# huttered40/capital

Hardware: AMD Instinct MI355X
Metric: TFLOP/s (whole node) Cholesky n=65536, algorithmic n^3/3, recursive cholinv factor(), inputs resident in HBM (higher is better)
Workload: dtype f64

## Files before the change

### capital_amd/src/alg/cholesky/cholinv/cholinv.h

```cpp
#ifndef CAPITAL_CHOLESKY_CHOLINV_H_
#define CAPITAL_CHOLESKY_CHOLINV_H_

#include "./../../alg.h"
#include "./../../matmult/summa/summa.h"
#include "./policy.h"

#pragma weak capi_dtrmm_thin
#pragma weak capi_dresid_ts

namespace cholesky {

template <class SerializePolicy = policy::cholinv::Serialize, class IntermediatesPolicy = policy::cholinv::SaveIntermediates,
          class BaseCasePolicy = policy::cholinv::NoReplication>
class cholinv : public SerializePolicy, public IntermediatesPolicy, public BaseCasePolicy {
public:
  using SP = SerializePolicy;
  using IP = IntermediatesPolicy;
  using BP = BaseCasePolicy;

  template <typename ScalarT, typename DimensionT>
  class info {
  public:
    using ScalarType = ScalarT;
    using DimensionType = DimensionT;
    using alg_type = cholinv<SerializePolicy, IntermediatesPolicy, BaseCasePolicy>;
    using SP = SerializePolicy;
    using IP = IntermediatesPolicy;
    using BP = BaseCasePolicy;
    info(const info& p) : complete_inv(p.complete_inv), split(p.split), bc_mult_dim(p.bc_mult_dim), dir(p.dir) {}
    info(info&& p) : complete_inv(p.complete_inv), split(p.split), bc_mult_dim(p.bc_mult_dim), dir(p.dir) {}
    info(DimensionType complete_inv, DimensionType split, DimensionType bc_mult_dim, char dir)
        : complete_inv(complete_inv), split(split), bc_mult_dim(bc_mult_dim), dir(dir) {}
    const DimensionType complete_inv, split, bc_mult_dim;
    const char dir;
    matrix<ScalarType, DimensionType, typename SerializePolicy::structure> R, Rinv;
    matrix<ScalarType, DimensionType, rect> Rfull, Rinvfull;
    matmult::arena work;
    DimensionType localDimension = 0, globalDimension = 0, trueLocalDimension = 0, trueGlobalDimension = 0, bcDimension = 0;
    int64_t num_base_cases = 0, num_levels = 0;
    bool solve_with_trsm = false;
    int potrf_info = 0;
    bool zeroed = false;
    const double* input = nullptr;
    DimensionType early_split = 0;
    DimensionType input_lead = 0;
    int la_depth = 0;
    bool factored = false, factored_trsm = false;
    DimensionType top_split = 0;
    matrix<ScalarType, DimensionType, rect> X, SolveW1, SolveW2, SolveRho, SolveD, SolveNorm2;
    std::vector<double> solve_residual_norms;
  };

  template <typename MatrixType, typename ArgType, typename CommType>
  static void factor(const MatrixType& A, ArgType& args, CommType&& CommInfo) {
    CRITTER_START(CI::factor);
    using U = typename ArgType::DimensionType;
    static_assert(std::is_same<typename MatrixType::StructureType, rect>::value, "cholinv::factor takes a rect-structured input block");
    if (!(args.split > 0) || args.dir != 'U') throw std::invalid_argument("cholinv: split > 0 and dir == 'U' required (cholinv.hpp:9)");
    if (CommInfo.d > 1 && CommInfo.d % CommInfo.c) throw std::invalid_argument("cholinv: c must divide d (or d == 1)");
    args.factored = false;
    args.factored_trsm = args.solve_with_trsm;
    args.top_split = 0;
    if (args.solve_with_trsm) { factor_trsm(A, args, CommInfo); args.factored = true; CRITTER_STOP(CI::factor); return; }
    const U localDimension = A.num_rows_local(), globalDimension = A.num_rows_global();
    CAPITAL_CHECK(capi_stream_select(capital::handle(), 0));
    CAPITAL_CHECK(capi_reset_info(capital::handle()));
    args.potrf_info = 0;
    args.R._register_(A.num_columns_global(), A.num_rows_global(), CommInfo.d, CommInfo.d);
    args.Rinv._register_(A.num_columns_global(), A.num_rows_global(), CommInfo.d, CommInfo.d);
    constexpr bool packed = !std::is_same<typename SP::structure, rect>::value;
    if (packed) {
      args.Rfull._register_(A.num_columns_global(), A.num_rows_global(), CommInfo.d, CommInfo.d);
      args.Rinvfull._register_(A.num_columns_global(), A.num_rows_global(), CommInfo.d, CommInfo.d);
    }
    double* R = packed ? args.Rfull.data() : (double*)args.R.data();
    double* Ri = packed ? args.Rinvfull.data() : (double*)args.Rinv.data();
    const U ld = localDimension;
    if (!args.zeroed) {
      capital::dev_zero(R, ld * ld);
      capital::dev_zero(Ri, ld * ld);
      args.zeroed = true;
    }
    U bcDimLocal = (U)(CommInfo.c * CommInfo.d);
    U bcMult = args.bc_mult_dim;
    if (bcMult < 0) { bcMult = -bcMult; for (U i = 0; i < bcMult; ++i) bcDimLocal *= 2; } else { for (U i = 0; i < bcMult; ++i) bcDimLocal /= 2; }
    bcDimLocal = std::max<U>(1, bcDimLocal);
    bcDimLocal = std::min<U>(localDimension, bcDimLocal);
    bcDimLocal = localDimension / bcDimLocal;
    args.localDimension = args.trueLocalDimension = localDimension;
    args.globalDimension = args.trueGlobalDimension = globalDimension;
    args.bcDimension = (U)CommInfo.d * bcDimLocal;
    args.num_base_cases = args.num_levels = 0;

    const U h1 = localDimension >> args.split;
    args.input = A.data();
    args.early_split = 0;
    const bool will_split = !(((localDimension * (U)CommInfo.d) <= args.bcDimension) || (h1 < args.split));
    args.input_lead = 0;
    args.top_split = will_split ? h1 : 0;
    if (will_split && h1 > 0 && h1 < ld) {
      capi_handle_t hh = capital::handle();
      U lead = h1;
      if (args.split == 1 && CommInfo.d == 1 && CommInfo.c == 1) while (lead >= 8192 && lead % 2 == 0 && (lead >> 1) * (U)CommInfo.d > args.bcDimension) lead >>= 1;
      CAPITAL_CHECK(capi_dlacpy(hh, 1, lead, lead, A.data(), ld, R, ld));
      CAPITAL_CHECK(capi_event_record(hh, EV_INPUT_HEAD));
      CAPITAL_CHECK(capi_stream_select(hh, 1));
      CAPITAL_CHECK(capi_event_wait(hh, EV_INPUT_HEAD));
      if (lead < h1) {
        CAPITAL_CHECK(capi_dlacpy(hh, 0, lead, h1 - lead, A.data() + (int64_t)lead * ld, ld, R + (int64_t)lead * ld, ld));
        CAPITAL_CHECK(capi_dlacpy(hh, 1, h1 - lead, h1 - lead, A.data() + lead + (int64_t)lead * ld, ld, R + lead + (int64_t)lead * ld, ld));
        CAPITAL_CHECK(capi_event_record(hh, EV_INPUT_MID));
        args.input_lead = lead;
      }
      CAPITAL_CHECK(capi_dlacpy(hh, 0, h1, ld - h1, A.data() + (int64_t)h1 * ld, ld, R + (int64_t)h1 * ld, ld));
      CAPITAL_CHECK(capi_dlacpy(hh, 1, ld - h1, ld - h1, A.data() + h1 + (int64_t)h1 * ld, ld, R + h1 + (int64_t)h1 * ld, ld));
      CAPITAL_CHECK(capi_event_record(hh, EV_INPUT_REST));
      CAPITAL_CHECK(capi_stream_select(hh, 0));
      args.early_split = h1;
    } else {
      CAPITAL_CHECK(capi_dlacpy(capital::handle(), 1, ld, ld, A.data(), ld, R, ld));
    }


    const bool single = (CommInfo.d == 1 && CommInfo.c == 1);
    capital::launch_rounds_scope rounds(true);
    const U h = localDimension - (localDimension >> args.split);
    const U agg = args.bcDimension;
    int64_t need = single ? (int64_t)h * h + (int64_t)h * h / 3 + 1024 : (int64_t)(CommInfo.d == 1 ? 8 : 12) * h * h + 4 * (int64_t)agg * agg + 4096;
    args.work.reserve(need);

    args.la_depth = 0;
    invoke(args, CommInfo, R, Ri, ld, (U)0, localDimension, globalDimension);

    if (packed) {
      const U e = args.early_split;
      if (e > 0) {
        pack_block(args, CAPI_UPPERTRI, R, (double*)args.R.data(), ld, e, ld, e, ld);
        pack_block(args, CAPI_UPPERTRI, Ri, (double*)args.Rinv.data(), ld, e, ld, e, ld);
        if (args.complete_inv) pack_block(args, CAPI_RECT, Ri, (double*)args.Rinv.data(), ld, e, ld, 0, e);
        CAPITAL_CHECK(capi_event_wait(capital::handle(), EV_EARLY_PACK));
      } else {
        serialize<uppertri, uppertri>::invoke(args.Rfull, args.R, 0, ld, 0, ld, 0, ld, 0, ld);
        serialize<uppertri, uppertri>::invoke(args.Rinvfull, args.Rinv, 0, ld, 0, ld, 0, ld, 0, ld);
      }
    }
    if (!IP::keep_arena) {
      capital::sync();
      args.work.release();
      if (packed) { args.Rfull._destroy_(); args.Rinvfull._destroy_(); args.zeroed = false; }
    }
    CRITTER_STOP(CI::factor);
    CAPITAL_CHECK(capi_get_info(capital::handle(), &args.potrf_info));
    const int failed = capital::ranks_with_nonzero(CommInfo.world, args.potrf_info);
    if (failed != 0)
      throw std::domain_error("cholinv::factor: the matrix is not positive definite (" +
                              (args.potrf_info != 0 ? "non-positive pivot " + std::to_string(args.potrf_info) + " of a diagonal block"
                                                    : std::string("reported by ") + std::to_string(failed) + " other rank(s) of the grid") +
                              "); R and Rinv are not valid");
    args.factored = true;
  }

  template <typename MatrixType, typename ArgType, typename CommType>
  static void solve(const MatrixType& A, const MatrixType& B, ArgType& args, CommType&& CommInfo, int refine = 1, bool residual = true) {
    static_assert(std::is_same<typename MatrixType::StructureType, rect>::value, "cholinv::solve takes rect-structured A and B");
    constexpr bool packed = !std::is_same<typename SP::structure, rect>::value;
    if (CommInfo.size > 1) throw std::logic_error("cholinv::solve is built for one rank: on a grid the factors are element-cyclic (factor there, solve on one rank)");
    if (!&capi_dtrmm_thin || !&capi_dresid_ts) throw std::logic_error("cholinv: this C-ABI library has no capi_dtrmm_thin / capi_dresid_ts: no solve");
    if (!args.factored || args.potrf_info != 0 || !args.R.filled() || (!args.solve_with_trsm && !args.Rinv.filled()))
      throw std::logic_error("cholinv::solve: factor() has not run or did not succeed: there are no valid factors to solve with");
    if (args.factored_trsm != args.solve_with_trsm)
      throw std::logic_error("cholinv::solve: solve_with_trsm was changed after factor(): the resident factors are those of the other mode; factor() again");
    const int64_t n = args.localDimension, r = B.num_columns_global();
    if (r < 1 || B.num_rows_global() != n || B.num_rows_local() != n || A.num_rows_local() != n || A.num_columns_local() != n || refine < 0)
      throw std::invalid_argument("cholinv::solve: B must be n x r with r >= 1 (matrix(r, n, 1, 1)), A the factored matrix, refine >= 0");
    const double* Rfullp = nullptr;
    if (args.solve_with_trsm) {
      Rfullp = packed ? (IP::keep_arena && args.Rfull.filled() ? args.Rfull.data() : nullptr) : (const double*)args.R.data();
      if (!Rfullp)
        throw std::logic_error("cholinv::solve: TRSM mode with Serialize + FlushIntermediates leaves only the packed R, and capi_dtrsm takes full "
                               "storage: use SaveIntermediates or NoSerialize with solve_with_trsm");
    }
    CRITTER_START(CI::solve);
    capi_handle_t h = capital::handle();
    CAPITAL_CHECK(capi_stream_select(h, 0));
    const int64_t W = CAPI_TS_MAX_RHS, h1 = args.top_split;
    const bool blocks = !args.solve_with_trsm && !args.complete_inv && h1 > 0 && h1 < n;
    if (args.X.filled() && args.X.num_columns_local() != r) args.X._destroy_();
    args.X._register_(r, n, 1, 1);
    args.SolveW1._register_(W, n, 1, 1);
    if (blocks) args.SolveW2._register_(W, n, 1, 1);
    if (refine > 0) { args.SolveRho._register_(W, n, 1, 1); args.SolveD._register_(W, n, 1, 1); }
    const double* Rp = (const double*)args.R.data();
    const double* Ip = args.solve_with_trsm ? nullptr : (const double*)args.Rinv.data();
    auto thin = [&](const double* F, int shape, int trans, int64_t i0, int64_t j0, int64_t m, int64_t k, int64_t rb, double alpha, const double* Bp,
                    double beta, double* Cp) {
      const double* Tp = packed ? F + j0 * (j0 + 1) / 2 + i0 : F + i0 + j0 * n;
      CAPITAL_CHECK(capi_dtrmm_thin(h, shape, trans, m, k, rb, alpha, Tp, packed ? 0 : n, packed ? j0 : 0, Bp, n, beta, Cp, n));
    };
    auto apply = [&](const double* Bi, double* Xo, int64_t rb) {
      double* w1 = args.SolveW1.data();
      if (args.solve_with_trsm) {
        CAPITAL_CHECK(capi_dlacpy(h, 0, n, rb, Bi, n, Xo, n));
        CAPITAL_CHECK(capi_dtrsm(h, CAPI_LEFT, CAPI_UPPER, CAPI_TRANS, CAPI_NONUNIT, n, rb, 1.0, Rfullp, n, Xo, n));
        CAPITAL_CHECK(capi_dtrsm(h, CAPI_LEFT, CAPI_UPPER, CAPI_NOTRANS, CAPI_NONUNIT, n, rb, 1.0, Rfullp, n, Xo, n));
      } else if (!blocks) {
        thin(Ip, CAPI_UPPERTRI, CAPI_TRANS, 0, 0, n, n, rb, 1.0, Bi, 0.0, w1);
        thin(Ip, CAPI_UPPERTRI, CAPI_NOTRANS, 0, 0, n, n, rb, 1.0, w1, 0.0, Xo);
      } else {
        const int64_t h2 = n - h1;
        double* w2 = args.SolveW2.data();
        thin(Ip, CAPI_UPPERTRI, CAPI_TRANS, 0, 0, h1, h1, rb, 1.0, Bi, 0.0, w1);
        CAPITAL_CHECK(capi_dlacpy(h, 0, h2, rb, Bi + h1, n, w2 + h1, n));
        thin(Rp, CAPI_RECT, CAPI_TRANS, 0, h1, h1, h2, rb, -1.0, w1, 1.0, w2 + h1);
        thin(Ip, CAPI_UPPERTRI, CAPI_TRANS, h1, h1, h2, h2, rb, 1.0, w2 + h1, 0.0, w1 + h1);
        thin(Ip, CAPI_UPPERTRI, CAPI_NOTRANS, h1, h1, h2, h2, rb, 1.0, w1 + h1, 0.0, Xo + h1);
        thin(Rp, CAPI_RECT, CAPI_NOTRANS, 0, h1, h1, h2, rb, -1.0, Xo + h1, 1.0, w1);
        thin(Ip, CAPI_UPPERTRI, CAPI_NOTRANS, 0, 0, h1, h1, rb, 1.0, w1, 0.0, Xo);
      }
    };
    for (int64_t j = 0; j < r; j += W) {
      const int64_t rb = std::min(W, r - j);
      double* Xj = args.X.data() + j * n;
      const double* Bj = B.data() + j * n;
      apply(Bj, Xj, rb);
      for (int it = 0; it < refine; ++it) {
        CAPITAL_CHECK(capi_dresid_ts(h, n, n, rb, A.data(), n, Xj, n, Bj, n, args.SolveRho.data(), n, nullptr));
        apply(args.SolveRho.data(), args.SolveD.data(), rb);
        CAPITAL_CHECK(capi_dgeadd(h, 0, n, rb, 1.0, args.SolveD.data(), n, 1.0, Xj, n));
      }
    }
    args.solve_residual_norms.clear();
    if (residual) {
      if (args.SolveNorm2.filled() && args.SolveNorm2.num_columns_local() != r) args.SolveNorm2._destroy_();
      args.SolveNorm2._register_(r, 1, 1, 1);
      for (int64_t j = 0; j < r; j += W)
        CAPITAL_CHECK(capi_dresid_ts(h, n, n, std::min(W, r - j), A.data(), n, args.X.data() + j * n, n, B.data() + j * n, n, nullptr, 0,
                                     args.SolveNorm2.data() + j));
      args.solve_residual_norms = args.SolveNorm2.to_host();
      for (double& v : args.solve_residual_norms) v = std::sqrt(v);
    }
    if (!IP::keep_arena) {
      capital::sync();
      args.SolveW1._destroy_(); args.SolveW2._destroy_(); args.SolveRho._destroy_(); args.SolveD._destroy_();
    }
    CRITTER_STOP(CI::solve);
  }

  template <typename MatrixType, typename ArgType, typename CommType>
  static void factor_trsm(const MatrixType& A, ArgType& args, CommType&& CommInfo) {
    using U = typename ArgType::DimensionType;
    capi_handle_t h = capital::handle();
    const U ld = A.num_rows_local();
    CAPITAL_CHECK(capi_stream_select(h, 0));
    CAPITAL_CHECK(capi_reset_info(h));
    args.potrf_info = 0;
    args.R._register_(A.num_columns_global(), A.num_rows_global(), CommInfo.d, CommInfo.d);
    constexpr bool packed = !std::is_same<typename SP::structure, rect>::value;
    if (packed) args.Rfull._register_(A.num_columns_global(), A.num_rows_global(), CommInfo.d, CommInfo.d);
    double* R = packed ? args.Rfull.data() : (double*)args.R.data();
    if (!args.zeroed) { capital::dev_zero(R, ld * ld); args.zeroed = true; }
    CAPITAL_CHECK(capi_dlacpy(h, 1, ld, ld, A.data(), ld, R, ld));
    U bcDimLocal = (U)(CommInfo.c * CommInfo.d), bcMult = args.bc_mult_dim;
    if (bcMult < 0) { bcMult = -bcMult; for (U i = 0; i < bcMult; ++i) bcDimLocal *= 2; } else { for (U i = 0; i < bcMult; ++i) bcDimLocal /= 2; }
    bcDimLocal = ld / std::min<U>(ld, std::max<U>(1, bcDimLocal));
    args.localDimension = args.trueLocalDimension = ld;
    args.globalDimension = args.trueGlobalDimension = A.num_rows_global();
    args.bcDimension = (U)CommInfo.d * bcDimLocal;
    args.num_base_cases = args.num_levels = 0;
    if (CommInfo.d == 1) {
      potrf_rec(args, R, ld, (U)0, ld);
    } else {
      const U hh = ld - (ld >> args.split);
      args.work.reserve((int64_t)32 * hh * hh + 4 * (int64_t)args.bcDimension * args.bcDimension + 4096);
      potrf_rec_grid(args, CommInfo, R, ld, (U)0, ld);
    }
    if (packed) serialize<uppertri, uppertri>::invoke(args.Rfull, args.R, 0, ld, 0, ld, 0, ld, 0, ld);
    CAPITAL_CHECK(capi_get_info(h, &args.potrf_info));
    const int failed = capital::ranks_with_nonzero(CommInfo.world, args.potrf_info);
    if (failed != 0)
      throw std::domain_error("cholinv::factor (TRSM mode): the matrix is not positive definite (non-positive pivot " + std::to_string(args.potrf_info) + " of a diagonal block)");
  }

  template <typename ArgType, typename CommType, typename U>
  static void potrf_rec_grid(ArgType& args, CommType&& t, double* R, U ld, U start, U dim) {
    using matmult::view;
    capi_handle_t h = capital::handle();
    matmult::arena& ws = args.work;
    const int64_t d = (int64_t)t.d, P = (int64_t)t.size, me = (int64_t)t.x + d * (int64_t)t.y;
    const U split1 = dim >> args.split;
    double* R11 = R + start + start * ld;
    if (((dim * (U)t.d) <= args.bcDimension) || (split1 < args.split)) {
      CRITTER_START(CI::factor_diag);
      const int64_t L = dim, agg = L * d;
      const int64_t span = ((start + dim) != args.trueLocalDimension) ? agg : agg - (args.trueLocalDimension * d - args.trueGlobalDimension);
      const int64_t mark = ws.top;
      double* mine = ws.take(L * L);
      double* blocked = ws.take(L * L * d * d);
      double* cyc = ws.take(agg * agg);
      CAPITAL_CHECK(capi_dlacpy(h, 0, L, L, R11, ld, mine, L));
      CAPITAL_CHECK(capi_allgather(t.slice, mine, blocked, L * L));
      util::block_to_cyclic_rect(blocked, cyc, L, L, d);
      CAPITAL_CHECK(capi_dpotrf(h, CAPI_UPPER, span, cyc, agg));
      CAPITAL_CHECK(capi_dtrizero(h, CAPI_UPPER, agg, cyc, agg));
      util::cyclic_to_block_rect(blocked, cyc, L, L, d);
      CAPITAL_CHECK(capi_dlacpy(h, 0, L, L, blocked + me * L * L, L, R11, ld));
      ws.top = mark;
      ++args.num_base_cases;
      CRITTER_STOP(CI::factor_diag);
      return;
    }
    ++args.num_levels;
    const U split2 = dim - split1;
    double* R12 = R + start + (start + split1) * ld;
    view A22{R + (start + split1) + (start + split1) * ld, ld, split2, split2};
    potrf_rec_grid(args, t, R, ld, start, split1);
    CRITTER_START(CI::trsm);
    const int64_t mark = ws.top;
    view W{ws.take((int64_t)split1 * split2), split1, split1, split2};
    {
      const int64_t L1 = split1, L2 = split2, S1 = L1 * d, S2 = L2 * d;
      const int64_t ncw = (((S2 + P - 1) / P) + 1) & ~(int64_t)1, S2p = ncw * P;
      const int64_t inner = ws.top;
      double* Rf = ws.take(S1 * S1);
      double* Xf = ws.take(S1 * S2p);
      double* mine = ws.take(L1 * std::max(L1, L2));
      double* blocked = ws.take(L1 * std::max(L1, L2) * d * d);
      CAPITAL_CHECK(capi_dlacpy(h, 0, L1, L1, R11, ld, mine, L1));
      CAPITAL_CHECK(capi_allgather(t.slice, mine, blocked, L1 * L1));
      util::block_to_cyclic_rect(blocked, Rf, L1, L1, d);
      CAPITAL_CHECK(capi_dlacpy(h, 0, L1, L2, R12, ld, mine, L1));
      CAPITAL_CHECK(capi_allgather(t.slice, mine, blocked, L1 * L2));
      if (S2p > S2) capital::dev_zero(Xf + S1 * S2, S1 * (S2p - S2));
      CAPITAL_CHECK(capi_block_to_cyclic_full(h, blocked, Xf, L1, L2, d));
      double* Xw = Xf + (int64_t)t.rank * ncw * S1;
      CAPITAL_CHECK(capi_dtrsm(h, CAPI_LEFT, CAPI_UPPER, CAPI_TRANS, CAPI_NONUNIT, S1, ncw, 1.0, Rf, S1, Xw, S1));
      CAPITAL_CHECK(capi_allgather(t.world, Xw, Xf, S1 * ncw));
      CAPITAL_CHECK(capi_cyclic_to_block(h, blocked, Xf, L1, L2, d));
      CAPITAL_CHECK(capi_dlacpy(h, 0, L1, L2, blocked + me * L1 * L2, L1, W.p, W.ld));
      CAPITAL_CHECK(capi_dlacpy(h, 0, L1, L2, W.p, W.ld, R12, ld));
      ws.top = inner;
    }
    CRITTER_STOP(CI::trsm);
    CRITTER_START(CI::tmu);
    {
      view Wx{ws.take(W.count()), split1, split1, split2};
      capital::dev_copy(Wx.p, W.p, W.count());
      util::transpose_raw(Wx.p, Wx.count(), ws.take(Wx.count()), t, matmult::summa::relay_space(t, Wx.count(), ws));
      matmult::summa::syrk(t, CAPI_UPPER, CAPI_TRANS, -1.0, W, Wx, 1.0, A22, ws);
    }
    ws.top = mark;
    CRITTER_STOP(CI::tmu);
    potrf_rec_grid(args, t, R, ld, start + split1, split2);
  }

  template <typename ArgType, typename U>
  static void potrf_rec(ArgType& args, double* R, U ld, U start, U dim) {
    capi_handle_t h = capital::handle();
    const U split1 = dim >> args.split;
    double* R11 = R + start + start * ld;
    if (dim <= args.bcDimension || split1 < args.split) {
      CRITTER_START(CI::factor_diag);
      CAPITAL_CHECK(capi_dpotrf(h, CAPI_UPPER, dim, R11, ld));
      CRITTER_STOP(CI::factor_diag);
      ++args.num_base_cases;
      return;
    }
    ++args.num_levels;
    const U split2 = dim - split1;
    double* R12 = R + start + (start + split1) * ld;
    double* R22 = R + (start + split1) + (start + split1) * ld;
    potrf_rec(args, R, ld, start, split1);
    CRITTER_START(CI::trsm);
    CAPITAL_CHECK(capi_dtrsm(h, CAPI_LEFT, CAPI_UPPER, CAPI_TRANS, CAPI_NONUNIT, split1, split2, 1.0, R11, ld, R12, ld));
    CRITTER_STOP(CI::trsm);
    CRITTER_START(CI::tmu);
    CAPITAL_CHECK(capi_dsyrk(h, CAPI_UPPER, CAPI_TRANS, split2, split1, -1.0, R12, ld, 1.0, R22, ld));
    CRITTER_STOP(CI::tmu);
    potrf_rec(args, R, ld, start + split1, split2);
  }

  template <typename ArgType, typename CommType>
  static matrix<typename ArgType::ScalarType, typename ArgType::DimensionType, rect> construct_R(ArgType& args, CommType&& CommInfo) {
    return construct(args.R, CommInfo);
  }
  template <typename ArgType, typename CommType>
  static matrix<typename ArgType::ScalarType, typename ArgType::DimensionType, rect> construct_Rinv(ArgType& args, CommType&& CommInfo) {
    if (args.solve_with_trsm) throw std::logic_error("cholinv: the TRSM mode forms no inverse (info::solve_with_trsm)");
    return construct(args.Rinv, CommInfo);
  }

private:
  static constexpr int EV_INPUT_HEAD = 1020, EV_INPUT_REST = 1021, EV_TOP_R12 = 1022, EV_EARLY_PACK = 1023, EV_INPUT_MID = 1019;
  static constexpr int EV_BC_POTRF = 1008, EV_BC_SCATTER = 1009;
  static constexpr int EV_LA_LEAD = 1010, EV_LA_REST = 1014, LA_STREAM0 = 2, LA_MAX_DEPTH = 2;
  static int64_t lookahead_min() {
    if (getenv("CAPITAL_NO_LOOKAHEAD")) return -1;
    const char* e = getenv("CAPITAL_LOOKAHEAD_MIN");
    if (e) return (int64_t)atoll(e);
    return getenv("CAPITAL_LOOKAHEAD") ? (int64_t)2048 : -1;
  }

  static int lookahead_depth() {
    const char* e = getenv("CAPITAL_LA_DEPTH");
    return e ? std::max(0, std::min(atoi(e), (int)LA_MAX_DEPTH)) : (int)LA_MAX_DEPTH;
  }

  template <typename ArgType>
  static void pack_block(ArgType&, int shape, const double* full, double* packed_dst, int64_t ld, int64_t x0, int64_t x1, int64_t y0,
                         int64_t y1) {
    CAPITAL_CHECK(capi_serialize_shape(capital::handle(), shape, CAPI_RECT, CAPI_UPPERTRI, full, ld, ld, packed_dst, ld, ld,
                                       x0, x1, y0, y1, x0, x1, y0, y1));
  }

  template <typename M, typename CommType>
  static matrix<typename M::ScalarType, typename M::DimensionType, rect> construct(M& src, CommType&& CommInfo) {
    const auto ld = src.num_rows_local();
    matrix<typename M::ScalarType, typename M::DimensionType, rect> ret(src.num_columns_global(), src.num_rows_global(), CommInfo.d, CommInfo.d);
    serialize<typename SP::structure, rect>::invoke(src, ret, 0, ld, 0, ld, 0, ld, 0, ld);
    return ret;
  }

  template <typename ArgType, typename CommType, typename U>
  static void invoke(ArgType& args, CommType&& t, double* R, double* Ri, U ld, U start, U localDim, U globalDim, int wait_ev = -1) {
    using matmult::view;
    capi_handle_t h = capital::handle();
    const U split1 = localDim >> args.split;
    if (((localDim * (U)t.d) <= args.bcDimension) || (split1 < args.split)) {
      if (wait_ev >= 0) CAPITAL_CHECK(capi_event_wait(h, wait_ev));
      CRITTER_START(CI::factor_diag);
      base_case(args, t, R, Ri, ld, start, localDim);
      CRITTER_STOP(CI::factor_diag);
      return;
    }
    ++args.num_levels;
    const U split2 = localDim - split1;
    const bool single = (t.d == 1 && t.c == 1);
    matmult::arena& ws = args.work;
    view R11i{Ri + start + start * ld, ld, split1, split1};
    view A12{R + start + (start + split1) * ld, ld, split1, split2};
    view A22{R + (start + split1) + (start + split1) * ld, ld, split2, split2};
    view R22i{Ri + (start + split1) + (start + split1) * ld, ld, split2, split2};
    view I12{Ri + start + (start + split1) * ld, ld, split1, split2};

    invoke(args, t, R, Ri, ld, start, split1, globalDim >> 1);
    if (wait_ev >= 0) CAPITAL_CHECK(capi_event_wait(h, wait_ev));
    if (start == 0 && args.input_lead > 0 && split1 == args.input_lead) CAPITAL_CHECK(capi_event_wait(h, EV_INPUT_MID));

    const bool top = (localDim == args.localDimension) && args.early_split == split1;
    if (top) CAPITAL_CHECK(capi_event_wait(h, EV_INPUT_REST));
    CRITTER_START(CI::trsm);
    int child_wait = -1;
    bool copy_deferred = false;
    const int64_t mark = ws.top;
    {
      view W{ws.take((int64_t)split1 * split2), split1, split1, split2};
      if (single) {
        CAPITAL_CHECK(capi_dtrmm_oop(h, CAPI_LEFT, CAPI_UPPER, CAPI_TRANS, CAPI_NONUNIT, split1, split2, 1.0, R11i.p, ld, A12.p, ld, W.p, W.ld));
      } else {
        view Tx{ws.take((int64_t)split1 * split1), split1, split1, split1};
        const int64_t np = matmult::summa::tri_count(split1);
        if ((t.x == t.y && !t.multipath) || !matmult::summa::packed_comm()) {
          CAPITAL_CHECK(capi_dlacpy(h, 0, split1, split1, R11i.p, ld, Tx.p, Tx.ld));
          util::transpose_raw(Tx.p, Tx.count(), ws.take(Tx.count()), t, matmult::summa::relay_space(t, Tx.count(), ws));
        } else if (t.x == t.y) {
          CAPITAL_CHECK(capi_dlacpy(h, 0, split1, split1, R11i.p, ld, Tx.p, Tx.ld));
          util::transpose_raw(nullptr, np, nullptr, t, matmult::summa::relay_space(t, np, ws));
        } else {
          double* pk = ws.take(np);
          matmult::summa::pack_tri(R11i, CAPI_UPPER, pk);
          util::transpose_raw(pk, np, ws.take(np), t, matmult::summa::relay_space(t, np, ws));
          matmult::summa::unpack_tri(pk, CAPI_UPPER, Tx);
        }
        matmult::summa::trmm(t, CAPI_LEFT, CAPI_UPPER, CAPI_TRANS, CAPI_NONUNIT, 1.0, Tx, A12, W, ws);
      }
      const U lead = split2 >> args.split;
      const bool a22_splits = !(((split2 * (U)t.d) <= args.bcDimension) || (lead < args.split));
      const bool la = single && a22_splits && lead > 0 && lookahead_min() >= 0 && (int64_t)split2 >= lookahead_min() && args.la_depth < lookahead_depth();
      const bool pack_now = top && !std::is_same<typename SP::structure, rect>::value;
      const bool copy_later = la && pack_now && !getenv("CAPITAL_PACK_AT_ONCE");
      if (!copy_later) CAPITAL_CHECK(capi_dlacpy(h, 0, split1, split2, W.p, W.ld, A12.p, ld));
      copy_deferred = copy_later;
      CRITTER_STOP(CI::trsm);
      auto early_pack = [&](int after_ev) {
        CAPITAL_CHECK(capi_stream_select(h, 1));
        CAPITAL_CHECK(capi_event_wait(h, after_ev));
        if (copy_later) CAPITAL_CHECK(capi_dlacpy(h, 0, split1, split2, W.p, W.ld, A12.p, ld));
        pack_block(args, CAPI_UPPERTRI, R, (double*)args.R.data(), ld, (U)0, split1, (U)0, split1);
        pack_block(args, CAPI_RECT, R, (double*)args.R.data(), ld, split1, ld, (U)0, split1);
        pack_block(args, CAPI_UPPERTRI, Ri, (double*)args.Rinv.data(), ld, (U)0, split1, (U)0, split1);
        CAPITAL_CHECK(capi_event_record(h, EV_EARLY_PACK));
        CAPITAL_CHECK(capi_stream_select(h, 0));
      };
      bool packed_early = false;

      CRITTER_START(CI::tmu);
      if (la) {
        const int depth = args.la_depth;
        const U rest = split2 - lead;
        double* Wr = W.p + (int64_t)lead * W.ld;
        CAPITAL_CHECK(capi_dgemmt(h, CAPI_UPPER, CAPI_TRANS, CAPI_NOTRANS, lead, split1, -1.0, W.p, W.ld, W.p, W.ld, 1.0, A22.p, ld));
        CAPITAL_CHECK(capi_event_record(h, EV_LA_LEAD + depth));
        CAPITAL_CHECK(capi_stream_select(h, LA_STREAM0 + depth));
        CAPITAL_CHECK(capi_event_wait(h, EV_LA_LEAD + depth));
        CAPITAL_CHECK(capi_dgemm(h, CAPI_TRANS, CAPI_NOTRANS, lead, rest, split1, -1.0, W.p, W.ld, Wr, W.ld, 1.0, A22.p + (int64_t)lead * ld, ld));
        CAPITAL_CHECK(capi_dgemmt(h, CAPI_UPPER, CAPI_TRANS, CAPI_NOTRANS, rest, split1, -1.0, Wr, W.ld, Wr, W.ld, 1.0,
                                  A22.p + lead + (int64_t)lead * ld, ld));
        CAPITAL_CHECK(capi_event_record(h, EV_LA_REST + depth));
        CAPITAL_CHECK(capi_stream_select(h, 0));
        child_wait = EV_LA_REST + depth;
        ++args.la_depth;
        if (pack_now && !getenv("CAPITAL_PACK_AT_ONCE")) { early_pack(EV_LA_REST + depth); packed_early = true; }
      } else if (single) {
        CAPITAL_CHECK(capi_dgemmt(h, CAPI_UPPER, CAPI_TRANS, CAPI_NOTRANS, split2, split1, -1.0, W.p, W.ld, W.p, W.ld, 1.0, A22.p, ld));
      } else {
        view Wx{ws.take(W.count()), split1, split1, split2};
        capital::dev_copy(Wx.p, W.p, W.count());
        util::transpose_raw(Wx.p, Wx.count(), ws.take(Wx.count()), t, matmult::summa::relay_space(t, Wx.count(), ws));
        matmult::summa::syrk(t, CAPI_UPPER, CAPI_TRANS, -1.0, W, Wx, 1.0, A22, ws);
      }
      if (pack_now && !packed_early) {
        CAPITAL_CHECK(capi_event_record(h, EV_TOP_R12));
        early_pack(EV_TOP_R12);
      }
      if (child_wait < 0) ws.top = mark;
      CRITTER_STOP(CI::tmu);
    }

    invoke(args, t, R, Ri, ld, start + split1, split2, split2 * (U)t.d, child_wait);
    if (child_wait >= 0) { --args.la_depth; ws.top = mark; }

    CRITTER_START(CI::tmu);
    if (!(!args.complete_inv && (globalDim == args.trueGlobalDimension))) {
      if (copy_deferred) CAPITAL_CHECK(capi_event_wait(h, EV_EARLY_PACK));
      const int64_t mark = ws.top;
      view W2{ws.take((int64_t)split1 * split2), split1, split1, split2};
      matmult::summa::trmm(t, CAPI_LEFT, CAPI_UPPER, CAPI_NOTRANS, CAPI_NONUNIT, 1.0, R11i, A12, W2, ws);
      if (single) {
        matmult::summa::trmm(t, CAPI_RIGHT, CAPI_UPPER, CAPI_NOTRANS, CAPI_NONUNIT, -1.0, R22i, W2, I12, ws);
      } else {
        view W3{ws.take(W2.count()), split1, split1, split2};
        matmult::summa::trmm(t, CAPI_RIGHT, CAPI_UPPER, CAPI_NOTRANS, CAPI_NONUNIT, -1.0, R22i, W2, W3, ws);
        CAPITAL_CHECK(capi_dlacpy(h, 0, split1, split2, W3.p, W3.ld, I12.p, ld));
      }
      ws.top = mark;
    }
    CRITTER_STOP(CI::tmu);
  }

  template <typename ArgType, typename CommType, typename U>
  static void base_case(ArgType& args, CommType&& t, double* R, double* Ri, U ld, U start, U localDim) {
    capi_handle_t h = capital::handle();
    ++args.num_base_cases;
    double* Rb = R + start + start * ld;
    double* Ib = Ri + start + start * ld;
    if (t.d == 1) {
      CAPITAL_CHECK(capi_dpotrf_trtri(h, localDim, Rb, ld, Ib, ld));
      return;
    }
    const int64_t d = (int64_t)t.d, L = (int64_t)localDim, agg = L * d;
    const int64_t span = ((start + localDim) != args.trueLocalDimension) ? agg : agg - (args.trueLocalDimension * d - args.trueGlobalDimension);
    constexpr bool packed_msg = !std::is_same<typename SP::structure, rect>::value;
    const int64_t piece = packed_msg ? L * (L + 1) / 2 : L * L;
    auto pack_piece = [&](const double* blk, double* dst) {
      if (packed_msg) CAPITAL_CHECK(capi_serialize_shape(h, CAPI_UPPERTRI, CAPI_RECT, CAPI_UPPERTRI, blk, ld, ld, dst, L, L, 0, L, 0, L, 0, L, 0, L));
      else CAPITAL_CHECK(capi_dlacpy(h, 0, L, L, blk, ld, dst, L));
    };
    auto unpack_piece = [&](const double* src, double* blk) {
      if (packed_msg) CAPITAL_CHECK(capi_serialize_shape(h, CAPI_UPPERTRI, CAPI_UPPERTRI, CAPI_RECT, src, L, L, blk, ld, ld, 0, L, 0, L, 0, L, 0, L));
      else CAPITAL_CHECK(capi_dlacpy(h, 0, L, L, src, L, blk, ld));
    };
    auto to_cyclic = [&](const double* blocked, double* cyc) {
      if (packed_msg) CAPITAL_CHECK(capi_block_to_cyclic_tri(h, blocked, cyc, L, d));
      else util::block_to_cyclic_rect(blocked, cyc, L, L, d);
    };
    auto to_blocked = [&](double* blocked, const double* cyc) {
      if (packed_msg) CAPITAL_CHECK(capi_cyclic_to_block_tri(h, blocked, cyc, L, d));
      else util::cyclic_to_block_rect(blocked, cyc, L, L, d);
    };
    matmult::arena& ws = args.work;
    const int64_t mark = ws.top;
    double* mine = ws.take(piece);
    double* minei = ws.take(piece);
    const int64_t me = (int64_t)t.x + d * (int64_t)t.y;
    const bool worker = BP::every_layer || t.z == 0;
    if (BP::gather_all) {
      double* blocked = ws.take(piece * d * d);
      double* cyc = ws.take(agg * agg);
      double* cyci = ws.take(agg * agg);
      if (worker) {
        pack_piece(Rb, mine);
        CAPITAL_CHECK(capi_allgather(t.slice, mine, blocked, piece));
        to_cyclic(blocked, cyc);
        capital::dev_zero(cyci, agg * agg);
        CAPITAL_CHECK(capi_dpotrf_trtri(h, span, cyc, agg, cyci, agg));
      }
      if (!BP::every_layer) {
        CAPITAL_CHECK(capi_bcast(t.depth, cyc, agg * agg, 0));
        CAPITAL_CHECK(capi_bcast(t.depth, cyci, agg * agg, 0));
      }
      to_blocked(blocked, cyc);
      unpack_piece(blocked + me * piece, Rb);
      to_blocked(blocked, cyci);
      unpack_piece(blocked + me * piece, Ib);
    } else {
      const bool root = worker && me == 0;
      double *blocked = nullptr, *cyc = nullptr, *cyci = nullptr;
      if (root) { blocked = ws.take(piece * d * d); cyc = ws.take(agg * agg); cyci = ws.take(agg * agg); }
      double* blockedi = (root && BP::overlap) ? ws.take(piece * d * d) : blocked;
      if (worker) {
        pack_piece(Rb, mine);
        CAPITAL_CHECK(capi_gather(t.slice, mine, blocked, piece, 0));
        if (!BP::overlap) {
          if (root) {
            to_cyclic(blocked, cyc);
            capital::dev_zero(cyci, agg * agg);
            CAPITAL_CHECK(capi_dpotrf_trtri(h, span, cyc, agg, cyci, agg));
            to_blocked(blocked, cyc);
          }
          CAPITAL_CHECK(capi_scatter(t.slice, blocked, mine, piece, 0));
          if (root) to_blocked(blocked, cyci);
          CAPITAL_CHECK(capi_scatter(t.slice, blocked, minei, piece, 0));
        } else {
          if (root) {
            to_cyclic(blocked, cyc);
            CAPITAL_CHECK(capi_dpotrf(h, CAPI_UPPER, span, cyc, agg));
            capital::dev_zero(cyci, agg * agg);
            CAPITAL_CHECK(capi_dlacpy(h, 1, span, span, cyc, agg, cyci, agg));
            to_blocked(blocked, cyc);
          }
          CAPITAL_CHECK(capi_event_record(h, EV_BC_POTRF));
          CAPITAL_CHECK(capi_stream_select(h, 1));
          CAPITAL_CHECK(capi_event_wait(h, EV_BC_POTRF));
          CAPITAL_CHECK(capi_scatter(t.slice, blocked, mine, piece, 0));
          CAPITAL_CHECK(capi_event_record(h, EV_BC_SCATTER));
          CAPITAL_CHECK(capi_stream_select(h, 0));
          if (root) {
            CAPITAL_CHECK(capi_dtrtri(h, CAPI_UPPER, CAPI_NONUNIT, span, cyci, agg));
            CAPITAL_CHECK(capi_dtrizero(h, CAPI_UPPER, agg, cyci, agg));
            to_blocked(blockedi, cyci);
          }
          CAPITAL_CHECK(capi_event_wait(h, EV_BC_SCATTER));
          CAPITAL_CHECK(capi_scatter(t.slice, blockedi, minei, piece, 0));
        }
      }
      CAPITAL_CHECK(capi_bcast(t.depth, mine, piece, 0));
      CAPITAL_CHECK(capi_bcast(t.depth, minei, piece, 0));
      unpack_piece(mine, Rb);
      unpack_piece(minei, Ib);
    }
    ws.top = mark;
  }
};

}

#endif
```

Before: 55.62.

## Read top R12 directly from input and pack it from W, plus early right-half pack

On a single device, the top-level off-diagonal block is no longer copied from the input into the R image. The trmm reads it straight from the input, and the packed R12 is serialized directly from the workspace W, so the write of W back into A12 can be skipped when the complete inverse is not needed. A second early pack is added for the right child's split: its R11/R12/Rinv blocks are packed on the side stream behind the lookahead update instead of at the end. The aim is to cut HBM copy traffic and move packing off the critical path. The cost is holding the workspace longer, which adds event waits and more stream coordination.

```diff
diff --git a/capital_amd/src/alg/cholesky/cholinv/cholinv.h b/capital_amd/src/alg/cholesky/cholinv/cholinv.h
--- a/capital_amd/src/alg/cholesky/cholinv/cholinv.h
+++ b/capital_amd/src/alg/cholesky/cholinv/cholinv.h
@@ -44,6 +44,8 @@
     const double* input = nullptr;
     DimensionType early_split = 0;
     DimensionType input_lead = 0;
+    bool r12_direct = false;
+    DimensionType right_split = 0;
     int la_depth = 0;
     bool factored = false, factored_trsm = false;
     DimensionType top_split = 0;
@@ -97,11 +99,14 @@
     args.early_split = 0;
     const bool will_split = !(((localDimension * (U)CommInfo.d) <= args.bcDimension) || (h1 < args.split));
     args.input_lead = 0;
+    args.r12_direct = false;
+    args.right_split = 0;
     args.top_split = will_split ? h1 : 0;
+    const bool single = (CommInfo.d == 1 && CommInfo.c == 1);
     if (will_split && h1 > 0 && h1 < ld) {
       capi_handle_t hh = capital::handle();
       U lead = h1;
-      if (args.split == 1 && CommInfo.d == 1 && CommInfo.c == 1) while (lead >= 8192 && lead % 2 == 0 && (lead >> 1) * (U)CommInfo.d > args.bcDimension) lead >>= 1;
+      if (args.split == 1 && single) while (lead >= 8192 && lead % 2 == 0 && (lead >> 1) * (U)CommInfo.d > args.bcDimension) lead >>= 1;
       CAPITAL_CHECK(capi_dlacpy(hh, 1, lead, lead, A.data(), ld, R, ld));
       CAPITAL_CHECK(capi_event_record(hh, EV_INPUT_HEAD));
       CAPITAL_CHECK(capi_stream_select(hh, 1));
@@ -112,7 +117,8 @@
         CAPITAL_CHECK(capi_event_record(hh, EV_INPUT_MID));
         args.input_lead = lead;
       }
-      CAPITAL_CHECK(capi_dlacpy(hh, 0, h1, ld - h1, A.data() + (int64_t)h1 * ld, ld, R + (int64_t)h1 * ld, ld));
+      args.r12_direct = single && !getenv("CAPITAL_R12_VIA_IMAGE");
+      if (!args.r12_direct) CAPITAL_CHECK(capi_dlacpy(hh, 0, h1, ld - h1, A.data() + (int64_t)h1 * ld, ld, R + (int64_t)h1 * ld, ld));
       CAPITAL_CHECK(capi_dlacpy(hh, 1, ld - h1, ld - h1, A.data() + h1 + (int64_t)h1 * ld, ld, R + h1 + (int64_t)h1 * ld, ld));
       CAPITAL_CHECK(capi_event_record(hh, EV_INPUT_REST));
       CAPITAL_CHECK(capi_stream_select(hh, 0));
@@ -122,7 +128,6 @@
     }
 
 
-    const bool single = (CommInfo.d == 1 && CommInfo.c == 1);
     capital::launch_rounds_scope rounds(true);
     const U h = localDimension - (localDimension >> args.split);
     const U agg = args.bcDimension;
@@ -134,11 +139,14 @@
 
     if (packed) {
       const U e = args.early_split;
+      const U f = e + args.right_split;
       if (e > 0) {
-        pack_block(args, CAPI_UPPERTRI, R, (double*)args.R.data(), ld, e, ld, e, ld);
-        pack_block(args, CAPI_UPPERTRI, Ri, (double*)args.Rinv.data(), ld, e, ld, e, ld);
+        pack_block(args, CAPI_UPPERTRI, R, (double*)args.R.data(), ld, f, ld, f, ld);
+        pack_block(args, CAPI_UPPERTRI, Ri, (double*)args.Rinv.data(), ld, f, ld, f, ld);
+        if (f > e) pack_block(args, CAPI_RECT, Ri, (double*)args.Rinv.data(), ld, f, ld, e, f);
         if (args.complete_inv) pack_block(args, CAPI_RECT, Ri, (double*)args.Rinv.data(), ld, e, ld, 0, e);
         CAPITAL_CHECK(capi_event_wait(capital::handle(), EV_EARLY_PACK));
+        if (f > e) CAPITAL_CHECK(capi_event_wait(capital::handle(), EV_RIGHT_PACK));
       } else {
         serialize<uppertri, uppertri>::invoke(args.Rfull, args.R, 0, ld, 0, ld, 0, ld, 0, ld);
         serialize<uppertri, uppertri>::invoke(args.Rinvfull, args.Rinv, 0, ld, 0, ld, 0, ld, 0, ld);
@@ -391,6 +399,7 @@
 
 private:
   static constexpr int EV_INPUT_HEAD = 1020, EV_INPUT_REST = 1021, EV_TOP_R12 = 1022, EV_EARLY_PACK = 1023, EV_INPUT_MID = 1019;
+  static constexpr int EV_RIGHT_R12 = 1006, EV_RIGHT_PACK = 1007;
   static constexpr int EV_BC_POTRF = 1008, EV_BC_SCATTER = 1009;
   static constexpr int EV_LA_LEAD = 1010, EV_LA_REST = 1014, LA_STREAM0 = 2, LA_MAX_DEPTH = 2;
   static int64_t lookahead_min() {
@@ -446,16 +455,22 @@
     if (wait_ev >= 0) CAPITAL_CHECK(capi_event_wait(h, wait_ev));
     if (start == 0 && args.input_lead > 0 && split1 == args.input_lead) CAPITAL_CHECK(capi_event_wait(h, EV_INPUT_MID));
 
+    constexpr bool packed = !std::is_same<typename SP::structure, rect>::value;
     const bool top = (localDim == args.localDimension) && args.early_split == split1;
+    const bool direct = top && args.r12_direct;
+    const bool right = single && packed && args.early_split > 0 && start == args.early_split && localDim == args.localDimension - start &&
+                       !getenv("CAPITAL_PACK_RIGHT_LATE");
+    if (right) args.right_split = split1;
     if (top) CAPITAL_CHECK(capi_event_wait(h, EV_INPUT_REST));
     CRITTER_START(CI::trsm);
     int child_wait = -1;
-    bool copy_deferred = false;
+    bool w_held = false;
     const int64_t mark = ws.top;
     {
       view W{ws.take((int64_t)split1 * split2), split1, split1, split2};
       if (single) {
-        CAPITAL_CHECK(capi_dtrmm_oop(h, CAPI_LEFT, CAPI_UPPER, CAPI_TRANS, CAPI_NONUNIT, split1, split2, 1.0, R11i.p, ld, A12.p, ld, W.p, W.ld));
+        CAPITAL_CHECK(capi_dtrmm_oop(h, CAPI_LEFT, CAPI_UPPER, CAPI_TRANS, CAPI_NONUNIT, split1, split2, 1.0, R11i.p, ld,
+                                     direct ? args.input + (int64_t)split1 * ld : A12.p, ld, W.p, W.ld));
       } else {
         view Tx{ws.take((int64_t)split1 * split1), split1, split1, split1};
         const int64_t np = matmult::summa::tri_count(split1);
@@ -476,19 +491,28 @@
       const U lead = split2 >> args.split;
       const bool a22_splits = !(((split2 * (U)t.d) <= args.bcDimension) || (lead < args.split));
       const bool la = single && a22_splits && lead > 0 && lookahead_min() >= 0 && (int64_t)split2 >= lookahead_min() && args.la_depth < lookahead_depth();
-      const bool pack_now = top && !std::is_same<typename SP::structure, rect>::value;
-      const bool copy_later = la && pack_now && !getenv("CAPITAL_PACK_AT_ONCE");
-      if (!copy_later) CAPITAL_CHECK(capi_dlacpy(h, 0, split1, split2, W.p, W.ld, A12.p, ld));
-      copy_deferred = copy_later;
+      const bool pack_now = (top && packed) || right;
+      const int ev_r12 = top ? EV_TOP_R12 : EV_RIGHT_R12, ev_pack = top ? EV_EARLY_PACK : EV_RIGHT_PACK;
+      const bool pack_behind_bulk = la && pack_now && !getenv("CAPITAL_PACK_AT_ONCE");
+      const bool pack_from_W = pack_now && direct;
+      const bool image_read = !pack_from_W || args.complete_inv;
+      const bool copy_later = image_read && top && pack_behind_bulk;
+      if (image_read && !copy_later) CAPITAL_CHECK(capi_dlacpy(h, 0, split1, split2, W.p, W.ld, A12.p, ld));
+      w_held = pack_from_W || copy_later;
       CRITTER_STOP(CI::trsm);
       auto early_pack = [&](int after_ev) {
+        const U mid = start + split1, end = start + localDim;
         CAPITAL_CHECK(capi_stream_select(h, 1));
         CAPITAL_CHECK(capi_event_wait(h, after_ev));
         if (copy_later) CAPITAL_CHECK(capi_dlacpy(h, 0, split1, split2, W.p, W.ld, A12.p, ld));
-        pack_block(args, CAPI_UPPERTRI, R, (double*)args.R.data(), ld, (U)0, split1, (U)0, split1);
-        pack_block(args, CAPI_RECT, R, (double*)args.R.data(), ld, split1, ld, (U)0, split1);
-        pack_block(args, CAPI_UPPERTRI, Ri, (double*)args.Rinv.data(), ld, (U)0, split1, (U)0, split1);
-        CAPITAL_CHECK(capi_event_record(h, EV_EARLY_PACK));
+        pack_block(args, CAPI_UPPERTRI, R, (double*)args.R.data(), ld, start, mid, start, mid);
+        if (pack_from_W)
+          CAPITAL_CHECK(capi_serialize_shape(h, CAPI_RECT, CAPI_RECT, CAPI_UPPERTRI, W.p, split2, split1, (double*)args.R.data(), ld, ld,
+                                             0, split2, 0, split1, mid, end, start, mid));
+        else
+          pack_block(args, CAPI_RECT, R, (double*)args.R.data(), ld, mid, end, start, mid);
+        pack_block(args, CAPI_UPPERTRI, Ri, (double*)args.Rinv.data(), ld, start, mid, start, mid);
+        CAPITAL_CHECK(capi_event_record(h, ev_pack));
         CAPITAL_CHECK(capi_stream_select(h, 0));
       };
       bool packed_early = false;
@@ -509,7 +533,7 @@
         CAPITAL_CHECK(capi_stream_select(h, 0));
         child_wait = EV_LA_REST + depth;
         ++args.la_depth;
-        if (pack_now && !getenv("CAPITAL_PACK_AT_ONCE")) { early_pack(EV_LA_REST + depth); packed_early = true; }
+        if (pack_behind_bulk) { early_pack(EV_LA_REST + depth); packed_early = true; }
       } else if (single) {
         CAPITAL_CHECK(capi_dgemmt(h, CAPI_UPPER, CAPI_TRANS, CAPI_NOTRANS, split2, split1, -1.0, W.p, W.ld, W.p, W.ld, 1.0, A22.p, ld));
       } else {
@@ -519,19 +543,20 @@
         matmult::summa::syrk(t, CAPI_UPPER, CAPI_TRANS, -1.0, W, Wx, 1.0, A22, ws);
       }
       if (pack_now && !packed_early) {
-        CAPITAL_CHECK(capi_event_record(h, EV_TOP_R12));
-        early_pack(EV_TOP_R12);
-      }
-      if (child_wait < 0) ws.top = mark;
+        CAPITAL_CHECK(capi_event_record(h, ev_r12));
+        early_pack(ev_r12);
+      }
+      if (child_wait < 0 && !w_held) ws.top = mark;
       CRITTER_STOP(CI::tmu);
     }
 
     invoke(args, t, R, Ri, ld, start + split1, split2, split2 * (U)t.d, child_wait);
-    if (child_wait >= 0) { --args.la_depth; ws.top = mark; }
+    if (w_held) CAPITAL_CHECK(capi_event_wait(h, EV_EARLY_PACK));
+    if (child_wait >= 0) --args.la_depth;
+    if (child_wait >= 0 || w_held) ws.top = mark;
 
     CRITTER_START(CI::tmu);
     if (!(!args.complete_inv && (globalDim == args.trueGlobalDimension))) {
-      if (copy_deferred) CAPITAL_CHECK(capi_event_wait(h, EV_EARLY_PACK));
       const int64_t mark = ws.top;
       view W2{ws.take((int64_t)split1 * split2), split1, split1, split2};
       matmult::summa::trmm(t, CAPI_LEFT, CAPI_UPPER, CAPI_NOTRANS, CAPI_NONUNIT, 1.0, R11i, A12, W2, ws);
```

Result: no change. 55.87 (median of 6 runs) (+0.4%).
